# ctSkennerton/crass

Hardware: AMD Instinct MI355X
Metric: reads/sec through DR search+recruit, 150bp synthetic, 1/2/4/8 MI355X (higher is better)
Workload: dtype u8; 1 GPU; 100000000 synthetic 150 bp reads, 50 seeded DRs, 1 % CRISPR reads (BASELINE.json configs[2]); pass1 + merge + pass2; total_reads=100000000, reads_per_gpu=100000000, read_len=150, n_dr=50, parallelism=read-shards x1, launcher=single context, pass1_found=563794, pass2_found=436000, patterns=13320, ac_states=0, filter_survivors=1705594, fast_filter=1, lds_automaton=2, merge_fallbacks=0

## Files before the change

crass_amd/build.py:

```python
import os
import shutil
import subprocess
import sys

HERE = os.path.dirname(os.path.abspath(__file__))
CSRC = os.path.join(HERE, "csrc")
LIB = os.path.join(HERE, "libcrass_hip.so")
SOURCES = ["kernels.hip", "pass2.hip", "sinks.hip", "dmerge.hip", "consensus.hip", "pack.hip", "fastx_scan.hip", "fastx_names.hip", "inflate.hip", "gunzip.hip", "engine.cpp", "merge.cpp", "ingest.cpp", "fastx_scan.cpp", "bgzf.cpp", "gunzip.cpp", "consensus.cpp", "group.cpp", "graph.cpp", "sdma.cpp", "pgzip.cpp"]
HEADERS = ["engine_internal.h", "dev_common.h", "comp_table.h", "devmem.h", "pack_text.h", "pack_launch.h", "fastx_scan.h", "fastx_launch.h", "fastx_names_launch.h", "inflate_core.h", "inflate_launch.h", "gunzip_core.h", "gunzip_launch.h", "consensus_internal.h", "merge.h", os.path.join("..", "..", "include", "crass_hip.h")]


def _hipcc():
    for cand in (os.environ.get("HIPCC"), shutil.which("hipcc"), "/opt/rocm/bin/hipcc"):
        if cand and os.path.exists(cand):
            return cand
    raise RuntimeError("hipcc not found: the MI355X engine cannot be built")


OBJ = os.path.join(CSRC, "_obj")
FLAGS = ["--offload-arch=gfx950", "-O3", "-std=c++17", "-ffp-contract=off", "-fPIC", "-Wall", "-Wno-unused-function"]
LIBS = ["-lz", "-lpthread", "-ldl"]


def _stale(target, deps):
    if not os.path.exists(target):
        return True
    t = os.path.getmtime(target)
    return any(os.path.getmtime(d) > t for d in deps)


def needs_build():
    return _stale(LIB, [os.path.join(CSRC, d) for d in SOURCES + HEADERS])


def build(force=False, verbose=False):
    if not force and not needs_build():
        return LIB
    os.makedirs(OBJ, exist_ok=True)
    hipcc = _hipcc()
    hdrs = [os.path.join(CSRC, h) for h in HEADERS]
    jobs = []
    objs = []
# ... 59 lines not shown
```

crass_amd/csrc/engine.cpp:

```cpp
#include "../../include/crass_hip.h"
#include "engine_internal.h"
#include "merge.h"
#include "pack_launch.h"
#include "fastx_launch.h"
#include "fastx_names_launch.h"
#include "inflate_launch.h"
#include "gunzip_launch.h"

#include <algorithm>
#include <atomic>
#include <chrono>
#include <cstdio>
#include <cstdlib>
#include <cstring>
#include <new>
#include <string>
#include <condition_variable>
#include <functional>
#include <mutex>
#include <thread>
#include <memory>
#include <utility>
#include <vector>

// ... 115 lines not shown
        if (want <= n && p) return hipSuccess;
        if (p) { (void)hipHostFree(p); p = nullptr; n = 0; }
        if (want == 0) want = 1;
        hipError_t e = hipHostMalloc((void **)&p, want * sizeof(T), hipHostMallocDefault);
        if (e == hipSuccess) n = want;
        return e;
    }
    void release() { if (p) (void)hipHostFree(p); p = nullptr; n = 0; }
};

}

struct EnvSwitches {
    bool no_lookback = false, no_pos_hints = false, merge_profile = false, no_lane_kernel = false;
    bool host_merge = false, no_speculation = false, exc_separate = false, dm_inject_fail = false, dm_init_late = false;
    bool no_presize = false;
    bool dd_full_table = false;
    bool no_device_view = false;
    bool force_device_view = false;
    bool no_dense_light = false;
    bool no_warm_launch = false;
    uint32_t view_group_cap = 32768;
    uint32_t view_sort_max = 2048;
    uint64_t test_bounds[4] = {0, 0, 0, 0};
    uint32_t row_cap = 256, dm_group_cap = 16384, surv_debug = 0;
    int stage_timing = -1;
    uint64_t pool_cap_bytes = 0;
    bool no_hint_filter = false;
    uint32_t wave_walk_min = 800;
    uint32_t long_min = 2048;
    uint64_t text_chunk_bytes = 64ull << 20;
    bool inflate_hbm_window = true;
    uint32_t hid_hash_bits = 64;
    uint32_t probe_blocks = 0;
    void read()
    {
        auto on = [](const char *n) { return getenv(n) != nullptr; };
        no_lookback = on("CRASS_NO_LOOKBACK"); no_pos_hints = on("CRASS_NO_POS_HINTS");
        merge_profile = on("CRASS_MERGE_PROFILE"); no_lane_kernel = on("CRASS_NO_LANE_KERNEL"); host_merge = on("CRASS_HOST_MERGE");
        no_speculation = on("CRASS_NO_SPECULATION"); exc_separate = on("CRASS_EXC_SEPARATE"); dm_init_late = on("CRASS_DM_INIT_LATE");
        dm_inject_fail = on("CRASS_DM_INJECT_FAIL"); no_presize = on("CRASS_NO_PRESIZE"); no_device_view = on("CRASS_NO_DEVICE_VIEW"); dd_full_table = on("CRASS_DD_FULL_TABLE"); force_device_view = on("CRASS_DEVICE_VIEW");
        view_group_cap = 32768; if (const char *e = getenv("CRASS_VIEW_GROUP_CAP")) view_group_cap = (uint32_t)std::max(1, atoi(e));
        view_sort_max = 2048; if (const char *e = getenv("CRASS_VIEW_SORT_MAX")) view_sort_max = (uint32_t)std::min(2048, std::max(64, atoi(e)));
        row_cap = 256; if (const char *e = getenv("CRASS_ROW_CAP")) row_cap = (uint32_t)std::max(1, atoi(e));
        dm_group_cap = 16384; if (const char *e = getenv("CRASS_DM_GROUP_CAP")) dm_group_cap = (uint32_t)std::max(1, atoi(e));
        surv_debug = 0; if (const char *e = getenv("CRASS_SURV_DEBUG")) surv_debug = (uint32_t)atoi(e);
        stage_timing = -1; if (const char *e = getenv("CRASS_STAGE_TIMING")) stage_timing = std::min(2, std::max(0, atoi(e)));
        for (auto &b : test_bounds) b = 0;
        if (const char *e = getenv("CRASS_TEST_BOUNDS")) { int k = 0; for (const char *q = e; *q && k < 4; k++) { test_bounds[k] = (uint64_t)atoll(q); while (*q && *q != ',') q++; if (*q == ',') q++; } }
        no_hint_filter = on("CRASS_NO_HINT_FILTER");
        wave_walk_min = 800; if (const char *e = getenv("CRASS_WAVE_WALK_MIN")) wave_walk_min = (uint32_t)std::max(0, atoi(e));
        long_min = 2048; if (const char *e = getenv("CRASS_LONG_MIN")) long_min = (uint32_t)std::max(0, atoi(e));
        no_warm_launch = getenv("CRASS_NO_WARM_LAUNCH") != nullptr;
        no_dense_light = getenv("CRASS_NO_DENSE_LIGHT") != nullptr;
        text_chunk_bytes = 64ull << 20; if (const char *e = getenv("CRASS_TEXT_CHUNK_BYTES")) text_chunk_bytes = (uint64_t)std::max(1ll, atoll(e));
        inflate_hbm_window = true; if (const char *e = getenv("CRASS_INFLATE_WINDOW")) inflate_hbm_window = strcmp(e, "lds") != 0;
        hid_hash_bits = 64; if (const char *e = getenv("CRASS_HID_TEST_HASH_BITS")) hid_hash_bits = (uint32_t)std::min(64, std::max(0, atoi(e)));
        probe_blocks = 0; if (const char *e = getenv("CRASS_PROBE_BLOCKS")) probe_blocks = (uint32_t)std::max(0, atoi(e));
        pool_cap_bytes = 0; if (const char *e = getenv("CRASS_POOL_CAP_MB")) pool_cap_bytes = (uint64_t)std::max(1ll, atoll(e)) << 20;
    }
};

struct crass_hip_ctx {
    crass_params prm{};
    EnvSwitches env;
    DevParams dp{};
    int device = 0;
    hipStream_t stream = nullptr;
    mutable int last_hip = 0;

    DevReads R{};
    bool have_reads = false;
    uint64_t read_base = 0;
    uint32_t max_len = 0;
    bool uniform = false;
    DevBuf<uint32_t> r_packed; DevBuf<uint64_t> r_word_off; DevBuf<uint32_t> r_lengths; DevBuf<uint64_t> r_header_id;
    DevBuf<uint32_t> r_exc_mask; DevBuf<uint64_t> r_exc_read; DevBuf<uint64_t> r_exc_off; DevBuf<uint8_t> r_exc_bytes;
    std::vector<uint64_t> h_exc_read;
    DevBuf<uint64_t> t_off; DevBuf<uint8_t> t_dev[2]; PinBuf<uint8_t> t_pin[2];
    hipEvent_t ev_t_copy[2] = {nullptr, nullptr}, ev_t_pack[2] = {nullptr, nullptr}, ev_t_time[2] = {nullptr, nullptr};
    float last_pack_ms = 0;
    DevBuf<uint8_t> x_raw, x_text; DevBuf<FxTile> x_tiles; DevBuf<FxBase> x_base; DevBuf<uint64_t> x_tot, x_rec_pos, x_seq_off;
    PinBuf<uint64_t> x_h_tot, x_h_rec_pos, x_h_seq_off;
    hipEvent_t ev_x_time[2] = {nullptr, nullptr};
    float last_scan_ms = 0;
    DevBuf<uint64_t> z_idx; DevBuf<uint32_t> z_reason; DevBuf<unsigned long long> z_verdict; DevBuf<uint8_t> z_raw, z_text;
    PinBuf<unsigned long long> z_h_verdict;
    hipEvent_t ev_z_time[2] = {nullptr, nullptr};
    float last_inflate_ms = 0;
    DevBuf<uint64_t> gz_a64, gz_b64; DevBuf<uint32_t> gz_a32, gz_b32; DevBuf<uint16_t> gz_sym; DevBuf<uint8_t> gz_win;
// ... 394 lines not shown
        case CRASS_ERR_IO: return "I/O error";
        case CRASS_ERR_RCCL: return "RCCL call failed (crass_hip_group_last_error())";
        default: return "unknown status";
    }
}

int crass_hip_last_hip_error(const crass_hip_ctx *ctx) { return ctx ? ctx->last_hip : 0; }
void *crass_hip_stream(const crass_hip_ctx *ctx) { return ctx ? (void *)ctx->stream : nullptr; }

int crass_hip_create(const crass_params *p, int device, crass_hip_ctx **out)
{
    if (!p || !out) return CRASS_ERR_INVALID_ARG;
    *out = nullptr;
    if (p->searchWindowLength < CRASS_HIP_MIN_WINDOW || p->searchWindowLength > CRASS_HIP_MAX_WINDOW) return CRASS_ERR_INVALID_ARG;
    if (p->lowDRsize < 8 || p->lowSpacerSize < 8) return CRASS_ERR_INVALID_ARG;
    if (p->lowDRsize >= p->highDRsize || p->lowSpacerSize >= p->highSpacerSize) return CRASS_ERR_INVALID_ARG;
    if (p->minNumRepeats < 2) return CRASS_ERR_INVALID_ARG;
    if (p->highDRsize > CRASS_HIP_MAX_DR) return CRASS_ERR_UNSUPPORTED;
    if (p->lowDRsize < 2 * p->searchWindowLength - 1) return CRASS_ERR_UNSUPPORTED;
    int ndev = 0;
    if (hipGetDeviceCount(&ndev) != hipSuccess || ndev <= 0 || device < 0 || device >= ndev) return CRASS_ERR_NO_DEVICE;
    crass_hip_ctx *c = new (std::nothrow) crass_hip_ctx();
    if (!c) return CRASS_ERR_OOM;
    c->prm = *p;
    c->device = device;
    c->dp.lowDR = p->lowDRsize; c->dp.highDR = p->highDRsize; c->dp.lowSp = p->lowSpacerSize; c->dp.highSp = p->highSpacerSize;
    c->dp.window = p->searchWindowLength; c->dp.minRepeats = p->minNumRepeats;
    uint32_t skips = p->lowDRsize - (2 * p->searchWindowLength - 1);
    if (skips < 1) skips = 1;
    c->dp.skips = skips;
    c->env.read();
    g_dev_cap.store(c->env.pool_cap_bytes, std::memory_order_relaxed);
    c->dp.debug_stop = c->env.surv_debug;
    if (c->env.stage_timing >= 0) c->timing_level = c->env.stage_timing;
    if (c->env.no_lookback) c->lb_on = false;
    c->dr_stride = (p->highDRsize + 15u) & ~15u;
    { const hipError_t he = hipSetDevice(device);
      if (he != hipSuccess) { fprintf(stderr, "[crass_hip] hipSetDevice(%d): %s\n", device, hipGetErrorString(he)); delete c; return CRASS_ERR_NO_DEVICE; } }
    if (const char *e = getenv("CRASS_WAIT")) {
        const unsigned f = !strcmp(e, "spin") ? hipDeviceScheduleSpin : !strcmp(e, "yield") ? hipDeviceScheduleYield : !strcmp(e, "block") ? hipDeviceScheduleBlockingSync : hipDeviceScheduleAuto;
        const hipError_t fe = hipSetDeviceFlags(f);
        if (fe != hipSuccess) fprintf(stderr, "[crass_hip] hipSetDeviceFlags(%s): %s\n", e, hipGetErrorString(fe));
    }
    if (getenv("CRASS_SURV_PROF")) {
        void *pp = nullptr;
        if (hipMalloc(&pp, (192 + 2 * 16384) * 8) == hipSuccess && hipMemset(pp, 0, (192 + 2 * 16384) * 8) == hipSuccess) {
            c->dp.prof = (unsigned long long *)pp;
            const unsigned long long big = ~0ull;
            (void)hipMemcpy(c->dp.prof + 188, &big, 8, hipMemcpyHostToDevice);
        }
    }
    for (hipStream_t *sp : {&c->stream, &c->copy_stream}) {
        const hipError_t he = hipStreamCreateWithFlags(sp, hipStreamNonBlocking);
        if (he != hipSuccess) { fprintf(stderr, "[crass_hip] hipStreamCreateWithFlags on device %d: %s\n", device, hipGetErrorString(he)); delete c; return CRASS_ERR_NO_DEVICE; }
    }
    for (auto &e : c->ev) if (hipEventCreate(&e) != hipSuccess) { delete c; return CRASS_ERR_HIP; }
    if (c->h_flags.ensure(8) != hipSuccess) { delete c; return CRASS_ERR_OOM; }
    memset(c->h_flags.p, 0, 32);
    c->poll_on = getenv("CRASS_NO_POLL") == nullptr;
    if (hipEventCreateWithFlags(&c->ev_gathered, hipEventDisableTiming) != hipSuccess) { delete c; return CRASS_ERR_HIP; }
    if (hipEventCreateWithFlags(&c->ev_premerge, hipEventDisableTiming) != hipSuccess) { delete c; return CRASS_ERR_HIP; }
    c->dma = sdma_create();
    if (c->dma && !getenv("CRASS_DX_PINNED")) {
        for (auto &d : c->dma_dx) d = sdma_create();
        c->dx_via_dma = c->dma_dx[0] && c->dma_dx[1] && c->dma_dx[2];
    }
    (void)warm_dmerge_module();
    *out = c;
    return CRASS_OK;
}

int crass_hip_stream_wait_event(crass_hip_ctx *c, void *event)
{
    if (!c || !event) return CRASS_ERR_INVALID_ARG;
    (void)hipSetDevice(c->device);
    HIPCHK(c, hipStreamWaitEvent(c->stream, (hipEvent_t)event, 0));
    return CRASS_OK;
}

int crass_hip_reload_env(crass_hip_ctx *c)
{
    if (!c) return CRASS_ERR_INVALID_ARG;
    c->env.read();
    g_dev_cap.store(c->env.pool_cap_bytes, std::memory_order_relaxed);
    c->dp.debug_stop = c->env.surv_debug;
    if (c->env.stage_timing >= 0) c->timing_level = c->env.stage_timing;
    c->lb_on = !c->env.no_lookback;
    return CRASS_OK;
}

int crass_hip_set_stage_timing(crass_hip_ctx *c, int level)
{
    if (!c || level < 0 || level > 2) return CRASS_ERR_INVALID_ARG;
    c->timing_level = level;
    return CRASS_OK;
}

int crass_hip_set_host_view(crass_hip_ctx *c, int light)
{
    if (!c || light < 0 || light > 1) return CRASS_ERR_INVALID_ARG;
    quiesce_worker(c);
    c->host_view_light = light != 0;
    if (c->host_view_light) c->dm.M.x_on = 0;
    return CRASS_OK;
}

int crass_hip_set_timing_focus(crass_hip_ctx *c, unsigned kernels)
{
    if (!c || kernels > 7u) return CRASS_ERR_INVALID_ARG;
    c->timing_focus = kernels;
    return CRASS_OK;
}

void crass_hip_destroy(crass_hip_ctx *c)
{
    if (!c) return;
    (void)hipSetDevice(c->device);
    quiesce_worker(c);
// ... 3582 lines not shown
```

crass_amd/csrc/engine_internal.h:

```cpp
#pragma once
#include <stdint.h>
#include <stddef.h>
#include <hip/hip_runtime.h>
#include "devmem.h"
#include "merge.h"

namespace crass {

struct DevReads {
    const uint32_t *packed;
    const uint64_t *word_off;
    const uint32_t *lengths;
    const uint64_t *header_id;
    const uint32_t *exc_mask;
    uint64_t n_reads;
    uint32_t stride_words;
    uint32_t uniform_len;
    const uint64_t *exc_read;
    const uint64_t *exc_off;
    const uint8_t  *exc_bytes;
    uint64_t n_exc;
    const uint64_t *pos_hint;
    const uint64_t *pos_hint_off;
    uint32_t wave_walk;
    uint32_t hint_all;
};

struct DevParams {
    uint32_t lowDR, highDR, lowSp, highSp, window, minRepeats;
    uint32_t skips;
    uint32_t debug_stop;
    uint32_t exc_survive;
    unsigned long long *prof;
};

struct SurvOut {
    uint32_t found;
    uint32_t n_ss;
    uint32_t repeat_len;
    uint32_t ss_off;
    uint16_t dr_len;
    uint8_t  low_lexi;
    uint8_t  err;
};

struct RecruitOut {
    uint32_t start, end;
    uint32_t token;
    uint16_t dr_len;
    uint8_t  low_lexi;
    uint8_t  pad;
};

struct DevAutomaton {
    const uint16_t *go16;
    const uint32_t *go32;
    const uint16_t *out_len;
    const uint32_t *out_pid;
    const uint16_t *go4;
    const uint32_t *go4w;
    uint32_t n_states;
    uint32_t n_sym1;
    uint8_t  sym[256];
    uint32_t acgt_ok;
    uint32_t max_pat_len;
// ... 326 lines not shown
```

crass_amd/csrc/kernels.hip:

```cpp
#include "dev_common.h"
#include "comp_table.h"
#include <type_traits>
#include <algorithm>

namespace crass {

static __constant__ CompTable c_comp = make_comp_table();

#define FG_WAVES 4

static __device__ __forceinline__ uint32_t lds_code(const uint32_t *w, uint32_t p, uint32_t mask)
{
    uint32_t wi = p >> 4, sh = (p & 15u) * 2u;
    uint64_t v = ((uint64_t)w[wi + 1] << 32) | w[wi];
    return (uint32_t)(v >> sh) & mask;
}

__global__ __launch_bounds__(FG_WAVES * WAVE) void k_filter_general(DevReads R, DevParams P, uint64_t *hitmask,
                                                                      uint32_t lds_words_per_wave)
{
    extern __shared__ __attribute__((aligned(16))) uint32_t fg_lds[];
    const int lane = threadIdx.x & 63;
    const int wave = threadIdx.x >> 6;
    uint32_t *words = fg_lds + (size_t)wave * lds_words_per_wave;
    const uint64_t n_words = (R.n_reads + 63) / 64;
    const uint32_t w = P.window;
    const uint32_t cmask = (1u << (2 * w)) - 1u;
    for (uint64_t mw = blockIdx.x * (uint64_t)FG_WAVES + wave; mw < n_words; mw += (uint64_t)gridDim.x * FG_WAVES) {
        uint64_t bits = 0;
        for (int k = 0; k < 64; k++) {
            uint64_t r = mw * 64 + k;
            if (r >= R.n_reads) break;
            if (!P.exc_survive && rd_is_exc(R, r)) continue;
            uint32_t L = rd_len(R, r);
// ... 2148 lines not shown
    const uint64_t v = ((uint64_t)ln_word(h, wi + 1) << 32) | ln_word(h, wi);
    return (uint32_t)(v >> sh) & h.cmask;
}
static __device__ __forceinline__ uint32_t ln_ss(const LaneRead &h, int k) { return h.ss[k * WAVE]; }
static __device__ __forceinline__ void ln_ss_set(LaneRead &h, int k, uint32_t v) { h.ss[k * WAVE] = (uint16_t)v; }

static __device__ __forceinline__ void ln_load128(const LaneRead &h, int start, uint64_t &lo, uint64_t &hi)
{
    const int wi = start >> 4;
    const uint32_t sh = (uint32_t)(start & 15) * 2u;
    const uint32_t a0 = ln_word(h, wi), a1 = ln_word(h, wi + 1), a2 = ln_word(h, wi + 2), a3 = ln_word(h, wi + 3), a4 = ln_word(h, wi + 4);
    const uint32_t y0 = __builtin_amdgcn_alignbit(a1, a0, sh), y1 = __builtin_amdgcn_alignbit(a2, a1, sh);
    const uint32_t y2 = __builtin_amdgcn_alignbit(a3, a2, sh), y3 = __builtin_amdgcn_alignbit(a4, a3, sh);
    lo = (uint64_t)y0 | ((uint64_t)y1 << 32); hi = (uint64_t)y2 | ((uint64_t)y3 << 32);
}
static __device__ __forceinline__ uint32_t ln_even_bits(uint64_t x)
{
    x &= 0x5555555555555555ull;
    x = (x | (x >> 1)) & 0x3333333333333333ull;
    x = (x | (x >> 2)) & 0x0F0F0F0F0F0F0F0Full;
    x = (x | (x >> 4)) & 0x00FF00FF00FF00FFull;
    x = (x | (x >> 8)) & 0x0000FFFF0000FFFFull;
    x = (x | (x >> 16)) & 0x00000000FFFFFFFFull;
    return (uint32_t)x;
}
static __device__ __forceinline__ void ln_planes(uint64_t lo, uint64_t hi, int n, uint64_t &p0, uint64_t &p1)
{
    p0 = (uint64_t)ln_even_bits(lo) | ((uint64_t)ln_even_bits(hi) << 32);
    p1 = (uint64_t)ln_even_bits(lo >> 1) | ((uint64_t)ln_even_bits(hi >> 1) << 32);
    const uint64_t m = n >= 64 ? ~0ull : ((1ull << n) - 1ull);
    p0 &= m; p1 &= m;
}

static __device__ int ln_find(const LaneRead &h, int begin, int end, int pat, int plen)
{
    if (end - begin <= 0 || plen <= 0 || plen > end - begin) return -1;
    const uint32_t sj = ln_code(h, pat);
    uint32_t code = ln_code(h, begin);
    const int top = 2 * (plen - 1);
    int nb = begin + plen;
    uint64_t buf = 0; int left = 0;
    for (int p = begin;; p++) {
        if (code == sj) return p;
        if (p + 1 + plen > end) return -1;
        if (left == 0) {
            const int wi = nb >> 4;
            const uint32_t sh = (uint32_t)(nb & 15) * 2u;
            const uint32_t a0 = ln_word(h, wi), a1 = ln_word(h, wi + 1), a2 = ln_word(h, wi + 2);
            buf = (uint64_t)__builtin_amdgcn_alignbit(a1, a0, sh) | ((uint64_t)__builtin_amdgcn_alignbit(a2, a1, sh) << 32);
            left = 32;
        }
        code = (code >> 2) | ((uint32_t)(buf & 3ull) << top);
        buf >>= 2; left--; nb++;
    }
}

static __device__ void ln_add(LaneRead &h, uint32_t i, uint32_t j)
{
    if (h.nss + 2 > h.cap) { h.punt = 1; return; }
    if (j >= (uint32_t)h.L) j = (uint32_t)h.L - 1;
    ln_ss_set(h, h.nss, i); ln_ss_set(h, h.nss + 1, j);
    h.nss += 2;
}

static __device__ void ln_scan_right(LaneRead &h, int pat, uint32_t pattern_length, uint32_t minSpacerLength, uint32_t scanRange)
{
    uint32_t last_repeat_index = ln_ss(h, h.nss - 2);
    uint32_t second_last_repeat_index = ln_ss(h, h.nss - 4);
    uint32_t repeat_spacing = last_repeat_index - second_last_repeat_index;
    const uint32_t read_length = (uint32_t)h.L;
    for (;;) {
        int candidate_repeat_index = (int)(last_repeat_index + repeat_spacing);
        uint32_t begin_search = (uint32_t)candidate_repeat_index - scanRange;
        uint32_t end_search = (uint32_t)candidate_repeat_index + pattern_length + scanRange;
        uint32_t scanRightMinBegin = last_repeat_index + pattern_length + minSpacerLength;
        if (begin_search < scanRightMinBegin) begin_search = scanRightMinBegin;
        if (begin_search > read_length - 1) return;
        if (end_search > read_length) end_search = read_length;
        if (begin_search >= end_search) return;
        int position = ln_find(h, (int)begin_search, (int)end_search, pat, (int)pattern_length);
        if (position < 0) return;
        ln_add(h, (uint32_t)position, (uint32_t)position + pattern_length - 1);
        if (h.punt) return;
        second_last_repeat_index = last_repeat_index;
        last_repeat_index = (uint32_t)position;
        repeat_spacing = last_repeat_index - second_last_repeat_index;
        if (repeat_spacing < (minSpacerLength + pattern_length)) return;
    }
}

static __device__ __forceinline__ int ln_run_up(uint64_t x0, uint64_t x1, int n)
{
    int r = x0 ? (__ffsll((unsigned long long)x0) - 1) >> 1 : (x1 ? 32 + ((__ffsll((unsigned long long)x1) - 1) >> 1) : 64);
    return r < n ? r : n;
}
static __device__ __forceinline__ int ln_run_down(uint64_t x0, uint64_t x1, int n)
{
    int r;
    if (n <= 32) { const uint64_t y = x0 << (64 - 2 * n); r = y ? __clzll((long long)y) >> 1 : n; }
    else {
        const uint64_t y1 = x1 << (64 - 2 * (n - 32));
        if (y1) r = __clzll((long long)y1) >> 1;
        else r = (n - 32) + (x0 ? __clzll((long long)x0) >> 1 : 32);
    }
    return r < n ? r : n;
}

static __device__ uint32_t ln_extend2(LaneRead &h, int searchWindowLength, int minSpacerLength)
{
    const int j = (int)ln_ss(h, 0), p = (int)ln_ss(h, 2), L = h.L, w = searchWindowLength;
    const int spacing = p - j;
    int max_right = spacing - minSpacerLength;
    if (max_right > L - (p + w)) max_right = L - (p + w);
// ... 135 lines not shown
    const int topbit = n - 1;
    for (int j = 0; j < m; j++) {
        const uint32_t c = ln_base(h, t0 + j);
        const WORD PMj = (pm0 & ((WORD)0 - (WORD)(c == 0))) | (pm1 & ((WORD)0 - (WORD)(c == 1))) |
                         (pm2 & ((WORD)0 - (WORD)(c == 2))) | (pm3 & ((WORD)0 - (WORD)(c == 3)));
        WORD TR = (WORD)((((WORD)~D0) & PMj) << 1) & PMold & ~(WORD)3;
        TR &= (WORD)0 - (WORD)(j >= 2);
        D0 = (WORD)((WORD)((WORD)(PMj & VP) + VP) ^ VP) | PMj | VN;
        D0 |= TR;
        WORD HP = VN | (WORD)~(D0 | VP);
        WORD HN = D0 & VP;
        dist += (int)((HP >> topbit) & 1) - (int)((HN >> topbit) & 1);
        HP = (WORD)(HP << 1) | (WORD)1;
        HN = (WORD)(HN << 1);
        VP = HN | (WORD)~(D0 | HP);
        VN = HP & D0;
        PMold = PMj;
    }
    return dist;
}

static __device__ int ln_distance(LaneRead &h, int s0, int n, int t0, int m, int stop_at)
{
    if (n > m) { int x = s0; s0 = t0; t0 = x; x = n; n = m; m = x; }
    if (n > 64) { h.punt = 1; return 0; }
    if (m <= 64) {
        uint64_t sl, sh, tl, th;
        ln_load128(h, s0, sl, sh); ln_load128(h, t0, tl, th);
        return ln_lev_regs<uint64_t>(sl, sh, n, tl, th, m, stop_at);
    }
    return (n <= 32) ? ln_lev_core<uint32_t>(h, s0, n, t0, m) : ln_lev_core<uint64_t>(h, s0, n, t0, m);
}

static __device__ float ln_similarity(LaneRead &h, int s0, int n, int t0, int m)
{
    float max_length = (float)(n > m ? n : m);
    if (n < 3 || m < 3) return 0.0f;
    const int d = ln_distance(h, s0, n, t0, m, -1);
    float edit_distance = (float)d;
    return (float)(1.0 - (double)(edit_distance / max_length));
}

static __device__ bool ln_similarity_above(LaneRead &h, int s0, int n, int t0, int m, double cut)
{
    if (n < 3 || m < 3) return 0.0 > cut;
    const float max_length = (float)(n > m ? n : m);
    int d_no = 0;
    while (d_no <= (n > m ? n : m) && (double)(float)(1.0 - (double)((float)d_no / max_length)) > cut) d_no++;
    const int d = ln_distance(h, s0, n, t0, m, d_no);
    if (h.punt) return false;
    return (double)(float)(1.0 - (double)((float)d / max_length)) > cut;
}

static __device__ int ln_qc(LaneRead &h, int minSpacerLength, int maxSpacerLength, uint32_t dbg = 0)
{
    if (dbg == 6) return 1;
    const int num_repeats = h.nss / 2;
    if (num_repeats < 2) return -1;
    uint32_t rep_len;
    const uint32_t rep_start = ln_ss(h, 0);
    if (!substr_len(h.L, rep_start, ln_ss(h, 1) - rep_start + 1, rep_len)) return -1;
    {
        int c0 = 0, c1 = 0, c2 = 0, c3 = 0;
        if (rep_len <= 64) {
            uint64_t lo, hi, p0, p1;
            ln_load128(h, (int)rep_start, lo, hi);
            ln_planes(lo, hi, (int)rep_len, p0, p1);
            c3 = __popcll(p0 & p1); c1 = __popcll(p0 & ~p1); c2 = __popcll(~p0 & p1); c0 = (int)rep_len - c1 - c2 - c3;
        } else
            for (uint32_t i = 0; i < rep_len; i++) { const uint32_t b = ln_base(h, (int)(rep_start + i)); c0 += (b == 0); c1 += (b == 1); c2 += (b == 2); c3 += (b == 3); }
        const int cut_off = (int)((double)(int)rep_len * 0.75);
        if (c0 > cut_off || c3 > cut_off || c2 > cut_off || c1 > cut_off) return 0;
    }
    if (dbg == 5) return 1;
    bool is_short = (2 > (num_repeats - 1));
    if (!is_short) {
        float ave_spacer_to_spacer_len_difference = 0.0f, ave_repeat_to_spacer_len_difference = 0.0f;
        float ave_spacer_to_spacer_difference = 0.0f, ave_repeat_to_spacer_difference = 0.0f;
        int min_spacer_length = 10000000, max_spacer_length = 0, num_compared = 0;
        const int nsp = num_repeats - 1;
        uint32_t cur_start = ln_ss(h, 1) + 1, cur_len;
        if (!substr_len(h.L, cur_start, ln_ss(h, 2) - cur_start, cur_len)) return -1;
        if (nsp == 2) {
            uint32_t nxt_start = ln_ss(h, 3) + 1, nxt_len;
            if (!substr_len(h.L, nxt_start, ln_ss(h, 4) - nxt_start, nxt_len)) return -1;
            const int mn = (int)(cur_len < nxt_len ? cur_len : nxt_len), mx = (int)(cur_len > nxt_len ? cur_len : nxt_len);
            if (mn < minSpacerLength || mx > maxSpacerLength) return 0;
            const bool a = ln_similarity_above(h, (int)cur_start, (int)cur_len, (int)nxt_start, (int)nxt_len, 0.82);
            if (h.punt) return 0;
            if (a) return 0;
            const bool b = ln_similarity_above(h, (int)rep_start, (int)rep_len, (int)cur_start, (int)cur_len, 0.82);
            if (h.punt) return 0;
            if (b) return 0;
            if ((int)fabsf(((float)cur_len - (float)nxt_len) / 1.0f) > 12) return 0;
            if ((int)fabsf(((float)rep_len - (float)cur_len) / 1.0f) > 30) return 0;
            return 1;
        }
        for (int i = 0; i < nsp; i++) {
            if ((int)cur_len < min_spacer_length) min_spacer_length = (int)cur_len;
            if ((int)cur_len > max_spacer_length) max_spacer_length = (int)cur_len;
            if (i + 1 < nsp) {
                uint32_t nxt_start = ln_ss(h, 2 * i + 3) + 1, nxt_len;
                if (!substr_len(h.L, nxt_start, ln_ss(h, 2 * i + 4) - nxt_start, nxt_len)) return -1;
                num_compared++;
                ave_repeat_to_spacer_difference += ln_similarity(h, (int)rep_start, (int)rep_len, (int)cur_start, (int)cur_len);
                float ss_diff = 0;
                ss_diff += ln_similarity(h, (int)cur_start, (int)cur_len, (int)nxt_start, (int)nxt_len);
                ave_spacer_to_spacer_difference += ss_diff;
                ave_spacer_to_spacer_len_difference += ((float)cur_len - (float)nxt_len);
                ave_repeat_to_spacer_len_difference += ((float)rep_len - (float)cur_len);
                cur_start = nxt_start; cur_len = nxt_len;
                if (h.punt) return 0;
            }
        }
        ave_spacer_to_spacer_difference /= (float)num_compared;
        ave_repeat_to_spacer_difference /= (float)num_compared;
        ave_spacer_to_spacer_len_difference /= (float)num_compared;
        ave_spacer_to_spacer_len_difference = fabsf(ave_spacer_to_spacer_len_difference);
        ave_repeat_to_spacer_len_difference /= (float)num_compared;
        ave_repeat_to_spacer_len_difference = fabsf(ave_repeat_to_spacer_len_difference);
        if (min_spacer_length < minSpacerLength) return 0;
        if (max_spacer_length > maxSpacerLength) return 0;
        if ((double)ave_spacer_to_spacer_difference > 0.82) return 0;
        if ((double)ave_repeat_to_spacer_difference > 0.82) return 0;
        if ((int)ave_spacer_to_spacer_len_difference > 12) return 0;
        if ((int)ave_repeat_to_spacer_len_difference > 30) return 0;
    }
    if (is_short) {
        uint32_t s = ln_ss(h, 1) + 1;
        uint32_t e = ln_ss(h, 2) - 1;
        uint32_t sp_len;
        if (!substr_len(h.L, s, e - s, sp_len)) return -1;
        if ((int)sp_len < minSpacerLength) return 0;
        if ((int)sp_len > maxSpacerLength) return 0;
        const bool too_similar = ln_similarity_above(h, (int)rep_start, (int)rep_len, (int)s, (int)sp_len, 0.82);
        if (h.punt) return 0;
        if (too_similar) return 0;
        int dlen = (int)sp_len - (int)rep_len;
        if (dlen < 0) dlen = -dlen;
        if (dlen > 30) return 0;
    }
    return 1;
}

struct QcTask { uint32_t a, b; };
struct QcPool {
    QcTask *task;
    uint8_t *res;
    uint32_t *cnt;
    const uint32_t *rows;
    uint32_t wave_words;
    uint32_t cap;
};
struct QcPending { int kind; uint32_t slot_a, slot_b; uint32_t cur_len, nxt_len, rep_len, sp_len; };

static __device__ uint32_t qc_enqueue_above(const QcPool &q, int s0, int n, int t0, int m, bool *now)
{
    *now = false;
    if (n < 3 || m < 3) { *now = 0.0 > 0.82; return 0xFFFFFFFFu; }
    if (n > m) { int x = s0; s0 = t0; t0 = x; x = n; n = m; m = x; }
    const float max_length = (float)m;
    int d_no = 0;
    while (d_no <= m && (double)(float)(1.0 - (double)((float)d_no / max_length)) > 0.82) d_no++;
    uint32_t slot;
    if (n <= 32) slot = atomicAdd(&q.cnt[0], 1u);
    else slot = q.cap - 1u - atomicAdd(&q.cnt[1], 1u);
    QcTask t;
    t.a = (uint32_t)threadIdx.x | ((uint32_t)s0 << 8) | ((uint32_t)n << 17) | ((uint32_t)d_no << 24);
    t.b = (uint32_t)t0 | ((uint32_t)m << 9);
    q.task[slot] = t;
    return slot;
}

template <typename WORD>
static __device__ __forceinline__ void qc_run_task(const QcPool &q, uint32_t slot)
{
    const QcTask t = q.task[slot];
    const uint32_t owner = t.a & 0xFFu;
    const int s0 = (int)((t.a >> 8) & 0x1FFu), n = (int)((t.a >> 17) & 0x7Fu), d_no = (int)(t.a >> 24);
    const int t0 = (int)(t.b & 0x1FFu), m = (int)(t.b >> 9);
    LaneRead ho;
    ho.w = q.rows + (size_t)(owner >> 6) * q.wave_words + (owner & 63u);
    uint64_t sl, sh, tl, th;
    ln_load128(ho, s0, sl, sh); ln_load128(ho, t0, tl, th);
    const int d = ln_lev_regs<WORD>(sl, sh, n, tl, th, m, d_no);
    q.res[slot] = (double)(float)(1.0 - (double)((float)d / (float)m)) > 0.82 ? 1 : 0;
}

static __device__ int qc_pool_begin(LaneRead &h, int minSpacerLength, int maxSpacerLength, uint32_t dbg, const QcPool &q, QcPending &pd)
{
    pd.kind = 0;
    const int num_repeats = h.nss / 2;
    if (dbg == 5 || dbg == 6 || num_repeats < 2 || num_repeats > 3) return ln_qc(h, minSpacerLength, maxSpacerLength, dbg);
    uint32_t rep_len;
    const uint32_t rep_start = ln_ss(h, 0);
    if (!substr_len(h.L, rep_start, ln_ss(h, 1) - rep_start + 1, rep_len)) return -1;
    if (rep_len > 64) return ln_qc(h, minSpacerLength, maxSpacerLength, dbg);
    {
        uint64_t lo, hi, p0, p1;
        ln_load128(h, (int)rep_start, lo, hi);
        ln_planes(lo, hi, (int)rep_len, p0, p1);
        const int c3 = __popcll(p0 & p1), c1 = __popcll(p0 & ~p1), c2 = __popcll(~p0 & p1), c0 = (int)rep_len - c1 - c2 - c3;
        const int cut_off = (int)((double)(int)rep_len * 0.75);
        if (c0 > cut_off || c3 > cut_off || c2 > cut_off || c1 > cut_off) return 0;
    }
    if (num_repeats == 3) {
        uint32_t cur_start = ln_ss(h, 1) + 1, cur_len;
        if (!substr_len(h.L, cur_start, ln_ss(h, 2) - cur_start, cur_len)) return -1;
        uint32_t nxt_start = ln_ss(h, 3) + 1, nxt_len;
        if (!substr_len(h.L, nxt_start, ln_ss(h, 4) - nxt_start, nxt_len)) return -1;
        const int mn = (int)(cur_len < nxt_len ? cur_len : nxt_len), mx = (int)(cur_len > nxt_len ? cur_len : nxt_len);
        if (mn < minSpacerLength || mx > maxSpacerLength) return 0;
        if (cur_len > 64 || nxt_len > 64) return ln_qc(h, minSpacerLength, maxSpacerLength, dbg);
        bool a_now, b_now;
        pd.slot_a = qc_enqueue_above(q, (int)cur_start, (int)cur_len, (int)nxt_start, (int)nxt_len, &a_now);
        if (pd.slot_a == 0xFFFFFFFFu && a_now) return 0;
        pd.slot_b = qc_enqueue_above(q, (int)rep_start, (int)rep_len, (int)cur_start, (int)cur_len, &b_now);
        if (pd.slot_b == 0xFFFFFFFFu && b_now) return 0;
        pd.kind = 3; pd.cur_len = cur_len; pd.nxt_len = nxt_len; pd.rep_len = rep_len;
        return 2;
    }
    uint32_t s = ln_ss(h, 1) + 1;
    uint32_t e = ln_ss(h, 2) - 1;
    uint32_t sp_len;
    if (!substr_len(h.L, s, e - s, sp_len)) return -1;
    if ((int)sp_len < minSpacerLength) return 0;
    if ((int)sp_len > maxSpacerLength) return 0;
    if (sp_len > 64) return ln_qc(h, minSpacerLength, maxSpacerLength, dbg);
    bool now;
    pd.slot_a = qc_enqueue_above(q, (int)rep_start, (int)rep_len, (int)s, (int)sp_len, &now);
    if (pd.slot_a == 0xFFFFFFFFu && now) return 0;
    pd.slot_b = 0xFFFFFFFFu;
    pd.kind = 2; pd.sp_len = sp_len; pd.rep_len = rep_len;
    return 2;
}
static __device__ int qc_pool_end(const QcPool &q, const QcPending &pd)
{
    const bool a = pd.slot_a != 0xFFFFFFFFu && q.res[pd.slot_a] != 0;
    if (pd.kind == 3) {
        if (a) return 0;
        const bool b = pd.slot_b != 0xFFFFFFFFu && q.res[pd.slot_b] != 0;
        if (b) return 0;
        if ((int)fabsf(((float)pd.cur_len - (float)pd.nxt_len) / 1.0f) > 12) return 0;
        if ((int)fabsf(((float)pd.rep_len - (float)pd.cur_len) / 1.0f) > 30) return 0;
        return 1;
    }
    if (a) return 0;
    int dlen = (int)pd.sp_len - (int)pd.rep_len;
    if (dlen < 0) dlen = -dlen;
    if (dlen > 30) return 0;
    return 1;
}

static __device__ int ln_search_core(LaneRead &h, const DevParams &o, uint64_t seed_hint, bool active, const QcPool &pool)
{
    const uint32_t seq_length = (uint32_t)h.L;
    const uint32_t skips = o.skips;
    int searchEnd = (int)(seq_length - o.lowDR - o.lowSp - o.window - 1);
    h.nss = 0;
    bool on_lattice = true;
    uint32_t lattice_i = 0;
    uint32_t j = 0;
    bool finished = !active || searchEnd < 0; int result = 0;
    for (;;) {
        bool ready = false, error = false, out_of_seeds = false;
        while (__any((int)(!finished && !ready && !out_of_seeds && !error))) {
            if (finished || ready || out_of_seeds || error) continue;
            while (on_lattice && j <= (uint32_t)searchEnd && lattice_i < 64 && !((seed_hint >> lattice_i) & 1ull)) { j += skips; lattice_i++; }
            if (j > (uint32_t)searchEnd) { out_of_seeds = true; continue; }
            if (on_lattice) lattice_i++;
            uint32_t beginSearch = j + o.lowDR + o.lowSp;
            uint32_t endSearch = j + o.highDR + o.highSp + o.window;
            if (endSearch >= seq_length) endSearch = seq_length - 1;
            if (endSearch < beginSearch) endSearch = beginSearch;
            if (beginSearch > seq_length) { error = true; continue; }
            int pos = ln_find(h, (int)beginSearch, (int)endSearch, (int)j, (int)o.window);
            if (o.debug_stop == 2) pos = -1;
            if (pos >= 0) {
                ln_add(h, j, j + o.window - 1);
                ln_add(h, (uint32_t)pos, (uint32_t)pos + o.window - 1);
                if (!h.punt) ln_scan_right(h, (int)j, o.window, o.lowSp, 24);
                if (h.punt) { finished = true; result = 0; continue; }
            }
            if ((uint32_t)(h.nss / 2) >= o.minRepeats) {
                uint32_t actual_repeat_length = ln_extend(h, (int)o.window, (int)o.lowSp);
                if (o.debug_stop != 3 && (actual_repeat_length >= o.lowDR) && (actual_repeat_length <= o.highDR)) { ready = true; continue; }
                j = ln_ss(h, h.nss - 1) - 1;
                on_lattice = false;
            }
            h.nss = 0;
            j = j + skips;
        }
        if (!finished && error) { finished = true; result = -1; }
        if (!finished && out_of_seeds) { finished = true; result = 0; }
        if (!__syncthreads_or((int)(!finished))) break;
        QcPending pd;
        pd.kind = 0;
        int qc = 0;
        if (!finished) qc = qc_pool_begin(h, (int)o.lowSp, (int)o.highSp, o.debug_stop, pool, pd);
        __syncthreads();
        {
            const uint32_t n32 = pool.cnt[0], n64 = pool.cnt[1];
            for (uint32_t t = threadIdx.x; t < n32; t += blockDim.x) qc_run_task<uint32_t>(pool, t);
            for (uint32_t t = blockDim.x - 1u - threadIdx.x; t < n64; t += blockDim.x) qc_run_task<uint64_t>(pool, pool.cap - 1u - t);
        }
        __syncthreads();
        if (threadIdx.x == 0) { pool.cnt[0] = 0u; pool.cnt[1] = 0u; }
        if (!finished) {
            if (qc == 2) qc = qc_pool_end(pool, pd);
            if (h.punt) { finished = true; result = 0; }
            else if (qc < 0) { finished = true; result = -1; }
            else if (qc) { finished = true; result = 1; }
            else {
                j = ln_ss(h, h.nss - 1) - 1;
// ... 307 lines not shown
```

Baseline: 29.96 billion reads/s.

## Use branch-free packed 2-bit SWAR search in ln_find and restructure lane QC

Replaces the per-position serial window search in ln_find with a SWAR routine. It processes a 128-bit packed chunk using alignbit and packed 16-bit min/multiply-add steps, which find the first match in two interleaved halves without per-position branches. The serial path stays available behind an environment flag and is still used for windows longer than 8. ln_qc is also folded into a single loop over similarity tests, and the queued QC fallback is forced inline, to cut code size and divergence. The cost is a fixed unrolled step count per chunk, which may waste work when a match would have been found early.

```diff
diff --git a/crass_amd/build.py b/crass_amd/build.py
--- a/crass_amd/build.py
+++ b/crass_amd/build.py
@@ -7,7 +7,7 @@
 CSRC = os.path.join(HERE, "csrc")
 LIB = os.path.join(HERE, "libcrass_hip.so")
 SOURCES = ["kernels.hip", "pass2.hip", "sinks.hip", "dmerge.hip", "consensus.hip", "pack.hip", "fastx_scan.hip", "fastx_names.hip", "inflate.hip", "gunzip.hip", "engine.cpp", "merge.cpp", "ingest.cpp", "fastx_scan.cpp", "bgzf.cpp", "gunzip.cpp", "consensus.cpp", "group.cpp", "graph.cpp", "sdma.cpp", "pgzip.cpp"]
-HEADERS = ["engine_internal.h", "dev_common.h", "comp_table.h", "devmem.h", "pack_text.h", "pack_launch.h", "fastx_scan.h", "fastx_launch.h", "fastx_names_launch.h", "inflate_core.h", "inflate_launch.h", "gunzip_core.h", "gunzip_launch.h", "consensus_internal.h", "merge.h", os.path.join("..", "..", "include", "crass_hip.h")]
+HEADERS = ["engine_internal.h", "dev_common.h", "comp_table.h", "devmem.h", "pack_text.h", "lane_find.h", "pack_launch.h", "fastx_scan.h", "fastx_launch.h", "fastx_names_launch.h", "inflate_core.h", "inflate_launch.h", "gunzip_core.h", "gunzip_launch.h", "consensus_internal.h", "merge.h", os.path.join("..", "..", "include", "crass_hip.h")]
 
 
 def _hipcc():
diff --git a/crass_amd/csrc/engine.cpp b/crass_amd/csrc/engine.cpp
--- a/crass_amd/csrc/engine.cpp
+++ b/crass_amd/csrc/engine.cpp
@@ -171,6 +171,7 @@
     uint64_t text_chunk_bytes = 64ull << 20;
     bool inflate_hbm_window = true;
     uint32_t hid_hash_bits = 64;
+    bool lane_find_serial = false;
     uint32_t probe_blocks = 0;
     void read()
     {
@@ -195,6 +196,7 @@
         text_chunk_bytes = 64ull << 20; if (const char *e = getenv("CRASS_TEXT_CHUNK_BYTES")) text_chunk_bytes = (uint64_t)std::max(1ll, atoll(e));
         inflate_hbm_window = true; if (const char *e = getenv("CRASS_INFLATE_WINDOW")) inflate_hbm_window = strcmp(e, "lds") != 0;
         hid_hash_bits = 64; if (const char *e = getenv("CRASS_HID_TEST_HASH_BITS")) hid_hash_bits = (uint32_t)std::min(64, std::max(0, atoi(e)));
+        lane_find_serial = false; if (const char *e = getenv("CRASS_LANE_FIND_SERIAL")) lane_find_serial = atoi(e) != 0;
         probe_blocks = 0; if (const char *e = getenv("CRASS_PROBE_BLOCKS")) probe_blocks = (uint32_t)std::max(0, atoi(e));
         pool_cap_bytes = 0; if (const char *e = getenv("CRASS_POOL_CAP_MB")) pool_cap_bytes = (uint64_t)std::max(1ll, atoll(e)) << 20;
     }
@@ -655,6 +657,7 @@
     c->env.read();
     g_dev_cap.store(c->env.pool_cap_bytes, std::memory_order_relaxed);
     c->dp.debug_stop = c->env.surv_debug;
+    c->dp.find_serial = c->env.lane_find_serial ? 1u : 0u;
     if (c->env.stage_timing >= 0) c->timing_level = c->env.stage_timing;
     if (c->env.no_lookback) c->lb_on = false;
     c->dr_stride = (p->highDRsize + 15u) & ~15u;
@@ -707,6 +710,7 @@
     c->env.read();
     g_dev_cap.store(c->env.pool_cap_bytes, std::memory_order_relaxed);
     c->dp.debug_stop = c->env.surv_debug;
+    c->dp.find_serial = c->env.lane_find_serial ? 1u : 0u;
     if (c->env.stage_timing >= 0) c->timing_level = c->env.stage_timing;
     c->lb_on = !c->env.no_lookback;
     return CRASS_OK;
diff --git a/crass_amd/csrc/engine_internal.h b/crass_amd/csrc/engine_internal.h
--- a/crass_amd/csrc/engine_internal.h
+++ b/crass_amd/csrc/engine_internal.h
@@ -31,6 +31,7 @@
     uint32_t skips;
     uint32_t debug_stop;
     uint32_t exc_survive;
+    uint32_t find_serial;
     unsigned long long *prof;
 };
 
diff --git a/crass_amd/csrc/kernels.hip b/crass_amd/csrc/kernels.hip
--- a/crass_amd/csrc/kernels.hip
+++ b/crass_amd/csrc/kernels.hip
@@ -1,5 +1,6 @@
 #include "dev_common.h"
 #include "comp_table.h"
+#include "lane_find.h"
 #include <type_traits>
 #include <algorithm>
 
@@ -2214,8 +2215,10 @@
     p0 &= m; p1 &= m;
 }
 
-static __device__ int ln_find(const LaneRead &h, int begin, int end, int pat, int plen)
-{
+static __device__ __noinline__ int ln_find_serial(const uint32_t *w, uint32_t cmask, int begin, int end, int pat, int plen)
+{
+    LaneRead h;
+    h.w = w; h.cmask = cmask;
     if (end - begin <= 0 || plen <= 0 || plen > end - begin) return -1;
     const uint32_t sj = ln_code(h, pat);
     uint32_t code = ln_code(h, begin);
@@ -2237,6 +2240,25 @@
     }
 }
 
+static __device__ __forceinline__ int ln_find(const LaneRead &h, int begin, int end, int pat, int plen, uint32_t serial)
+{
+    if (serial || plen > 8) return ln_find_serial(h.w, h.cmask, begin, end, pat, plen);
+    int left = (end - begin <= 0 || plen <= 0 || plen > end - begin) ? 0 : end - plen - begin + 1;
+    const uint32_t sj = ln_code(h, pat);
+    const int chunk = 64 - plen + 1;
+    int found = -1;
+    while (__any((int)(left > 0))) {
+        uint64_t lo, hi;
+        ln_load128(h, begin, lo, hi);
+        const int n = left < chunk ? left : chunk;
+        const int t = find_packed_steps(lo, hi, sj, plen, n, __any((int)(n > kLaneFindShortNpos)) != 0);
+        if (t >= 0) { found = begin + t; left = 0; }
+        else if (left > chunk) { left -= chunk; begin += chunk; }
+        else left = 0;
+    }
+    return found;
+}
+
 static __device__ void ln_add(LaneRead &h, uint32_t i, uint32_t j)
 {
     if (h.nss + 2 > h.cap) { h.punt = 1; return; }
@@ -2245,7 +2267,7 @@
     h.nss += 2;
 }
 
-static __device__ void ln_scan_right(LaneRead &h, int pat, uint32_t pattern_length, uint32_t minSpacerLength, uint32_t scanRange)
+static __device__ void ln_scan_right(LaneRead &h, int pat, uint32_t pattern_length, uint32_t minSpacerLength, uint32_t scanRange, uint32_t find_serial)
 {
     uint32_t last_repeat_index = ln_ss(h, h.nss - 2);
     uint32_t second_last_repeat_index = ln_ss(h, h.nss - 4);
@@ -2260,7 +2282,7 @@
         if (begin_search > read_length - 1) return;
         if (end_search > read_length) end_search = read_length;
         if (begin_search >= end_search) return;
-        int position = ln_find(h, (int)begin_search, (int)end_search, pat, (int)pattern_length);
+        int position = ln_find(h, (int)begin_search, (int)end_search, pat, (int)pattern_length, find_serial);
         if (position < 0) return;
         ln_add(h, (uint32_t)position, (uint32_t)position + pattern_length - 1);
         if (h.punt) return;
@@ -2462,27 +2484,7 @@
     return (n <= 32) ? ln_lev_core<uint32_t>(h, s0, n, t0, m) : ln_lev_core<uint64_t>(h, s0, n, t0, m);
 }
 
-static __device__ float ln_similarity(LaneRead &h, int s0, int n, int t0, int m)
-{
-    float max_length = (float)(n > m ? n : m);
-    if (n < 3 || m < 3) return 0.0f;
-    const int d = ln_distance(h, s0, n, t0, m, -1);
-    float edit_distance = (float)d;
-    return (float)(1.0 - (double)(edit_distance / max_length));
-}
-
-static __device__ bool ln_similarity_above(LaneRead &h, int s0, int n, int t0, int m, double cut)
-{
-    if (n < 3 || m < 3) return 0.0 > cut;
-    const float max_length = (float)(n > m ? n : m);
-    int d_no = 0;
-    while (d_no <= (n > m ? n : m) && (double)(float)(1.0 - (double)((float)d_no / max_length)) > cut) d_no++;
-    const int d = ln_distance(h, s0, n, t0, m, d_no);
-    if (h.punt) return false;
-    return (double)(float)(1.0 - (double)((float)d / max_length)) > cut;
-}
-
-static __device__ int ln_qc(LaneRead &h, int minSpacerLength, int maxSpacerLength, uint32_t dbg = 0)
+static __device__ __forceinline__ int ln_qc(LaneRead &h, int minSpacerLength, int maxSpacerLength, uint32_t dbg)
 {
     if (dbg == 6) return 1;
     const int num_repeats = h.nss / 2;
@@ -2503,73 +2505,90 @@
         if (c0 > cut_off || c3 > cut_off || c2 > cut_off || c1 > cut_off) return 0;
     }
     if (dbg == 5) return 1;
-    bool is_short = (2 > (num_repeats - 1));
-    if (!is_short) {
-        float ave_spacer_to_spacer_len_difference = 0.0f, ave_repeat_to_spacer_len_difference = 0.0f;
-        float ave_spacer_to_spacer_difference = 0.0f, ave_repeat_to_spacer_difference = 0.0f;
-        int min_spacer_length = 10000000, max_spacer_length = 0, num_compared = 0;
-        const int nsp = num_repeats - 1;
-        uint32_t cur_start = ln_ss(h, 1) + 1, cur_len;
+    const int nsp = num_repeats - 1;
+    const int mode = nsp < 2 ? 0 : (nsp == 2 ? 1 : 2);
+    float ave_spacer_to_spacer_len_difference = 0.0f, ave_repeat_to_spacer_len_difference = 0.0f;
+    float ave_spacer_to_spacer_difference = 0.0f, ave_repeat_to_spacer_difference = 0.0f;
+    int min_spacer_length = 10000000, max_spacer_length = 0, num_compared = 0;
+    uint32_t cur_start = ln_ss(h, 1) + 1, cur_len = 0, nxt_start = 0, nxt_len = 0;
+    if (mode == 0) {
+        const uint32_t e = ln_ss(h, 2) - 1;
+        if (!substr_len(h.L, cur_start, e - cur_start, cur_len)) return -1;
+        if ((int)cur_len < minSpacerLength) return 0;
+        if ((int)cur_len > maxSpacerLength) return 0;
+    } else {
         if (!substr_len(h.L, cur_start, ln_ss(h, 2) - cur_start, cur_len)) return -1;
-        if (nsp == 2) {
-            uint32_t nxt_start = ln_ss(h, 3) + 1, nxt_len;
+        if (mode == 1) {
+            nxt_start = ln_ss(h, 3) + 1;
             if (!substr_len(h.L, nxt_start, ln_ss(h, 4) - nxt_start, nxt_len)) return -1;
             const int mn = (int)(cur_len < nxt_len ? cur_len : nxt_len), mx = (int)(cur_len > nxt_len ? cur_len : nxt_len);
             if (mn < minSpacerLength || mx > maxSpacerLength) return 0;
-            const bool a = ln_similarity_above(h, (int)cur_start, (int)cur_len, (int)nxt_start, (int)nxt_len, 0.82);
+        }
+    }
+    const int n_tests = mode == 0 ? 1 : (mode == 1 ? 2 : 2 * (nsp - 1));
+    for (int k = 0; k < n_tests; k++) {
+        bool rep_vs_cur;
+        if (mode == 2) {
+            rep_vs_cur = !(k & 1);
+            if (rep_vs_cur) {
+                if ((int)cur_len < min_spacer_length) min_spacer_length = (int)cur_len;
+                if ((int)cur_len > max_spacer_length) max_spacer_length = (int)cur_len;
+                nxt_start = ln_ss(h, k + 3) + 1;
+                if (!substr_len(h.L, nxt_start, ln_ss(h, k + 4) - nxt_start, nxt_len)) return -1;
+                num_compared++;
+            }
+        } else rep_vs_cur = mode == 0 || k == 1;
+        const int s0 = rep_vs_cur ? (int)rep_start : (int)cur_start, n = rep_vs_cur ? (int)rep_len : (int)cur_len;
+        const int t0 = rep_vs_cur ? (int)cur_start : (int)nxt_start, m = rep_vs_cur ? (int)cur_len : (int)nxt_len;
+        float sim = 0.0f;
+        if (!(n < 3 || m < 3)) {
+            const float max_length = (float)(n > m ? n : m);
+            int stop_at = -1;
+            if (mode != 2) {
+                stop_at = 0;
+                while (stop_at <= (n > m ? n : m) && (double)(float)(1.0 - (double)((float)stop_at / max_length)) > 0.82) stop_at++;
+            }
+            const int d = ln_distance(h, s0, n, t0, m, stop_at);
             if (h.punt) return 0;
-            if (a) return 0;
-            const bool b = ln_similarity_above(h, (int)rep_start, (int)rep_len, (int)cur_start, (int)cur_len, 0.82);
-            if (h.punt) return 0;
-            if (b) return 0;
-            if ((int)fabsf(((float)cur_len - (float)nxt_len) / 1.0f) > 12) return 0;
-            if ((int)fabsf(((float)rep_len - (float)cur_len) / 1.0f) > 30) return 0;
-            return 1;
-        }
-        for (int i = 0; i < nsp; i++) {
-            if ((int)cur_len < min_spacer_length) min_spacer_length = (int)cur_len;
-            if ((int)cur_len > max_spacer_length) max_spacer_length = (int)cur_len;
-            if (i + 1 < nsp) {
-                uint32_t nxt_start = ln_ss(h, 2 * i + 3) + 1, nxt_len;
-                if (!substr_len(h.L, nxt_start, ln_ss(h, 2 * i + 4) - nxt_start, nxt_len)) return -1;
-                num_compared++;
-                ave_repeat_to_spacer_difference += ln_similarity(h, (int)rep_start, (int)rep_len, (int)cur_start, (int)cur_len);
-                float ss_diff = 0;
-                ss_diff += ln_similarity(h, (int)cur_start, (int)cur_len, (int)nxt_start, (int)nxt_len);
-                ave_spacer_to_spacer_difference += ss_diff;
-                ave_spacer_to_spacer_len_difference += ((float)cur_len - (float)nxt_len);
-                ave_repeat_to_spacer_len_difference += ((float)rep_len - (float)cur_len);
-                cur_start = nxt_start; cur_len = nxt_len;
-                if (h.punt) return 0;
-            }
-        }
-        ave_spacer_to_spacer_difference /= (float)num_compared;
-        ave_repeat_to_spacer_difference /= (float)num_compared;
-        ave_spacer_to_spacer_len_difference /= (float)num_compared;
-        ave_spacer_to_spacer_len_difference = fabsf(ave_spacer_to_spacer_len_difference);
-        ave_repeat_to_spacer_len_difference /= (float)num_compared;
-        ave_repeat_to_spacer_len_difference = fabsf(ave_repeat_to_spacer_len_difference);
-        if (min_spacer_length < minSpacerLength) return 0;
-        if (max_spacer_length > maxSpacerLength) return 0;
-        if ((double)ave_spacer_to_spacer_difference > 0.82) return 0;
-        if ((double)ave_repeat_to_spacer_difference > 0.82) return 0;
-        if ((int)ave_spacer_to_spacer_len_difference > 12) return 0;
-        if ((int)ave_repeat_to_spacer_len_difference > 30) return 0;
-    }
-    if (is_short) {
-        uint32_t s = ln_ss(h, 1) + 1;
-        uint32_t e = ln_ss(h, 2) - 1;
-        uint32_t sp_len;
-        if (!substr_len(h.L, s, e - s, sp_len)) return -1;
-        if ((int)sp_len < minSpacerLength) return 0;
-        if ((int)sp_len > maxSpacerLength) return 0;
-        const bool too_similar = ln_similarity_above(h, (int)rep_start, (int)rep_len, (int)s, (int)sp_len, 0.82);
-        if (h.punt) return 0;
-        if (too_similar) return 0;
-        int dlen = (int)sp_len - (int)rep_len;
+            sim = (float)(1.0 - (double)((float)d / max_length));
+        }
+        if (mode != 2) {
+            if ((double)sim > 0.82) return 0;
+        } else if (rep_vs_cur) ave_repeat_to_spacer_difference += sim;
+        else {
+            float ss_diff = 0;
+            ss_diff += sim;
+            ave_spacer_to_spacer_difference += ss_diff;
+            ave_spacer_to_spacer_len_difference += ((float)cur_len - (float)nxt_len);
+            ave_repeat_to_spacer_len_difference += ((float)rep_len - (float)cur_len);
+            cur_start = nxt_start; cur_len = nxt_len;
+        }
+    }
+    if (mode == 0) {
+        int dlen = (int)cur_len - (int)rep_len;
         if (dlen < 0) dlen = -dlen;
         if (dlen > 30) return 0;
-    }
+        return 1;
+    }
+    if (mode == 1) {
+        if ((int)fabsf(((float)cur_len - (float)nxt_len) / 1.0f) > 12) return 0;
+        if ((int)fabsf(((float)rep_len - (float)cur_len) / 1.0f) > 30) return 0;
+        return 1;
+    }
+    if ((int)cur_len < min_spacer_length) min_spacer_length = (int)cur_len;
+    if ((int)cur_len > max_spacer_length) max_spacer_length = (int)cur_len;
+    ave_spacer_to_spacer_difference /= (float)num_compared;
+    ave_repeat_to_spacer_difference /= (float)num_compared;
+    ave_spacer_to_spacer_len_difference /= (float)num_compared;
+    ave_spacer_to_spacer_len_difference = fabsf(ave_spacer_to_spacer_len_difference);
+    ave_repeat_to_spacer_len_difference /= (float)num_compared;
+    ave_repeat_to_spacer_len_difference = fabsf(ave_repeat_to_spacer_len_difference);
+    if (min_spacer_length < minSpacerLength) return 0;
+    if (max_spacer_length > maxSpacerLength) return 0;
+    if ((double)ave_spacer_to_spacer_difference > 0.82) return 0;
+    if ((double)ave_repeat_to_spacer_difference > 0.82) return 0;
+    if ((int)ave_spacer_to_spacer_len_difference > 12) return 0;
+    if ((int)ave_repeat_to_spacer_len_difference > 30) return 0;
     return 1;
 }
 
@@ -2617,15 +2636,15 @@
     q.res[slot] = (double)(float)(1.0 - (double)((float)d / (float)m)) > 0.82 ? 1 : 0;
 }
 
-static __device__ int qc_pool_begin(LaneRead &h, int minSpacerLength, int maxSpacerLength, uint32_t dbg, const QcPool &q, QcPending &pd)
+static __device__ __forceinline__ int qc_pool_begin_queued(LaneRead &h, int minSpacerLength, int maxSpacerLength, uint32_t dbg, const QcPool &q, QcPending &pd)
 {
     pd.kind = 0;
     const int num_repeats = h.nss / 2;
-    if (dbg == 5 || dbg == 6 || num_repeats < 2 || num_repeats > 3) return ln_qc(h, minSpacerLength, maxSpacerLength, dbg);
+    if (dbg == 5 || dbg == 6 || num_repeats < 2 || num_repeats > 3) return 3;
     uint32_t rep_len;
     const uint32_t rep_start = ln_ss(h, 0);
     if (!substr_len(h.L, rep_start, ln_ss(h, 1) - rep_start + 1, rep_len)) return -1;
-    if (rep_len > 64) return ln_qc(h, minSpacerLength, maxSpacerLength, dbg);
+    if (rep_len > 64) return 3;
     {
         uint64_t lo, hi, p0, p1;
         ln_load128(h, (int)rep_start, lo, hi);
@@ -2641,7 +2660,7 @@
         if (!substr_len(h.L, nxt_start, ln_ss(h, 4) - nxt_start, nxt_len)) return -1;
         const int mn = (int)(cur_len < nxt_len ? cur_len : nxt_len), mx = (int)(cur_len > nxt_len ? cur_len : nxt_len);
         if (mn < minSpacerLength || mx > maxSpacerLength) return 0;
-        if (cur_len > 64 || nxt_len > 64) return ln_qc(h, minSpacerLength, maxSpacerLength, dbg);
+        if (cur_len > 64 || nxt_len > 64) return 3;
         bool a_now, b_now;
         pd.slot_a = qc_enqueue_above(q, (int)cur_start, (int)cur_len, (int)nxt_start, (int)nxt_len, &a_now);
         if (pd.slot_a == 0xFFFFFFFFu && a_now) return 0;
@@ -2656,13 +2675,19 @@
     if (!substr_len(h.L, s, e - s, sp_len)) return -1;
     if ((int)sp_len < minSpacerLength) return 0;
     if ((int)sp_len > maxSpacerLength) return 0;
-    if (sp_len > 64) return ln_qc(h, minSpacerLength, maxSpacerLength, dbg);
+    if (sp_len > 64) return 3;
     bool now;
     pd.slot_a = qc_enqueue_above(q, (int)rep_start, (int)rep_len, (int)s, (int)sp_len, &now);
     if (pd.slot_a == 0xFFFFFFFFu && now) return 0;
     pd.slot_b = 0xFFFFFFFFu;
     pd.kind = 2; pd.sp_len = sp_len; pd.rep_len = rep_len;
     return 2;
+}
+static __device__ __forceinline__ int qc_pool_begin(LaneRead &h, int minSpacerLength, int maxSpacerLength, uint32_t dbg, const QcPool &q, QcPending &pd)
+{
+    const int r = qc_pool_begin_queued(h, minSpacerLength, maxSpacerLength, dbg, q, pd);
+    if (__builtin_expect(r == 3, 0)) return ln_qc(h, minSpacerLength, maxSpacerLength, dbg);
+    return r;
 }
 static __device__ int qc_pool_end(const QcPool &q, const QcPending &pd)
 {
@@ -2704,12 +2729,12 @@
             if (endSearch >= seq_length) endSearch = seq_length - 1;
             if (endSearch < beginSearch) endSearch = beginSearch;
             if (beginSearch > seq_length) { error = true; continue; }
-            int pos = ln_find(h, (int)beginSearch, (int)endSearch, (int)j, (int)o.window);
+            int pos = ln_find(h, (int)beginSearch, (int)endSearch, (int)j, (int)o.window, o.find_serial);
             if (o.debug_stop == 2) pos = -1;
             if (pos >= 0) {
                 ln_add(h, j, j + o.window - 1);
                 ln_add(h, (uint32_t)pos, (uint32_t)pos + o.window - 1);
-                if (!h.punt) ln_scan_right(h, (int)j, o.window, o.lowSp, 24);
+                if (!h.punt) ln_scan_right(h, (int)j, o.window, o.lowSp, 24, o.find_serial);
                 if (h.punt) { finished = true; result = 0; continue; }
             }
             if ((uint32_t)(h.nss / 2) >= o.minRepeats) {
diff --git a/crass_amd/csrc/lane_find.h b/crass_amd/csrc/lane_find.h
--- /dev/null
+++ b/crass_amd/csrc/lane_find.h
@@ -0,0 +1,75 @@
+#pragma once
+#include <stdint.h>
+
+#ifndef CRASS_HD
+#ifdef __HIPCC__
+#define CRASS_HD __host__ __device__
+#else
+#define CRASS_HD
+#endif
+#endif
+
+#ifdef __HIPCC__
+#define CRASS_LF_UNROLL _Pragma("unroll")
+#else
+#define CRASS_LF_UNROLL
+#endif
+
+namespace crass {
+
+CRASS_HD inline uint32_t lf_alignbit(uint32_t hi, uint32_t lo, uint32_t sh)
+{
+#if defined(__HIP_DEVICE_COMPILE__)
+    return __builtin_amdgcn_alignbit(hi, lo, sh);
+#else
+    return sh ? (lo >> sh) | (hi << (32u - sh)) : lo;
+#endif
+}
+
+CRASS_HD inline uint32_t lf_step(uint32_t acc, uint32_t x)
+{
+#if defined(__HIP_DEVICE_COMPILE__)
+    typedef unsigned short u16x2 __attribute__((ext_vector_type(2)));
+    uint32_t nz;
+    asm("v_pk_min_u16 %0, %1, %2" : "=v"(nz) : "v"(x), "v"(0x00010001u));
+    const u16x2 z = __builtin_bit_cast(u16x2, nz);
+    return __builtin_bit_cast(uint32_t, (u16x2)(__builtin_bit_cast(u16x2, acc) * z + z));
+#else
+    const uint32_t nl = (x & 0xFFFFu) ? 1u : 0u, nh = (x >> 16) ? 1u : 0u;
+    return ((((acc & 0xFFFFu) + 1u) * nl) & 0xFFFFu) | (((((acc >> 16) + 1u) * nh) & 0xFFFFu) << 16);
+#endif
+}
+
+constexpr int kLaneFindSteps = 32;
+constexpr int kLaneFindShortNpos = 49, kLaneFindShortSteps = 25;
+
+CRASS_HD inline int find_packed_steps(uint64_t lo, uint64_t hi, uint32_t code, int plen, int npos, bool all_steps)
+{
+    const uint32_t w[5] = {(uint32_t)lo, (uint32_t)(lo >> 32), (uint32_t)hi, (uint32_t)(hi >> 32), 0u};
+    const uint32_t m = (1u << (2 * plen)) - 1u;
+    const uint32_t mask2 = m | (m << 16), code2 = (code & m) | ((code & m) << 16);
+    uint32_t acc = 0;
+    if (all_steps) {
+CRASS_LF_UNROLL
+        for (int i = kLaneFindSteps - 1; i >= kLaneFindShortSteps; i--) {
+            const int k = i >> 3, t = i & 7;
+            acc = lf_step(acc, (lf_alignbit(w[k + 1], w[k], 2u * (uint32_t)t) ^ code2) & mask2);
+        }
+    }
+CRASS_LF_UNROLL
+    for (int i = kLaneFindShortSteps - 1; i >= 0; i--) {
+        const int k = i >> 3, t = i & 7;
+        acc = lf_step(acc, (lf_alignbit(w[k + 1], w[k], 2u * (uint32_t)t) ^ code2) & mask2);
+    }
+    const uint32_t cl = acc & 0xFFFFu, ch = acc >> 16;
+    const uint32_t ol = ((cl >> 3) << 4) + (cl & 7u), oh = ((ch >> 3) << 4) + (ch & 7u) + 8u;
+    const uint32_t o = ol < oh ? ol : oh;
+    return (int)o < npos ? (int)o : -1;
+}
+
+CRASS_HD inline int find_packed(uint64_t lo, uint64_t hi, uint32_t code, int plen, int npos)
+{
+    return find_packed_steps(lo, hi, code, plen, npos, true);
+}
+
+}
```

Measured after the change: 30.50 billion reads/s, median of 6. 1.8% higher.
